# KumarRobotics/top_down_renderer

Hardware: AMD Instinct MI355X
Metric: particle-updates/sec (render+score+resample) (higher is better)
Workload: dtype f32

## Files before the change

### include/tdr.h

```cpp
#ifndef TDR_H_
#define TDR_H_

#include <stddef.h>
#include <stdint.h>

#ifdef __cplusplus
extern "C" {
#endif

#define TDR_OK 0
#define TDR_ERR_ARG (-1)
#define TDR_ERR_HIP (-2)
#define TDR_ERR_NOMEM (-3)

#define TDR_MAX_CLASSES 15
#define TDR_ST_FIELDS 7
enum { TDR_ST_INIT_X = 0, TDR_ST_INIT_Y = 1, TDR_ST_DX = 2, TDR_ST_DY = 3, TDR_ST_THETA = 4, TDR_ST_SCALE = 5,
       TDR_ST_HAVE_INIT = 6 };

typedef struct tdr_state {
  float init_x_px, init_y_px, dx_m, dy_m, theta, scale;
  uint8_t have_init;
  uint8_t pad_[3];
} tdr_state;
// ... 114 lines not shown
int tdr_k_score_cart_init(const tdr_map_desc* map, const float* scan_pk, int rows, int cols, float res,
                          const tdr_filter_params* fp, float* st, int64_t cap, int64_t n, int64_t n_total,
                          float* workspace, void* stream);

int tdr_k_propagate(float* st, int64_t cap, int64_t n, float* last_dist, float tx, float ty, float omega,
                    int scale_freeze, float pos_cov, float theta_cov, const float* z4, uint64_t seed, uint64_t step,
                    int64_t index_base, void* stream);
void* tdr_rng_create(uint32_t seed);
void tdr_rng_destroy(void* rng);
float tdr_rng_uniform_host(void* rng);
int tdr_propagate_normals_host(void* rng, int64_t n, int scale_freeze, float* z4_out);
#define TDR_RNG_STATE_WORDS 640
size_t tdr_rng_dev_workspace_bytes(int64_t n);
int tdr_k_rng_propagate_normals(uint32_t* state, int64_t n, int64_t lo, int64_t hi, int scale_freeze, float* z4_out,
                                void* workspace, void* stream);
int tdr_k_rng_uniform(uint32_t* state, float* out_dev, void* stream);
int tdr_rng_get_state_host(void* rng, uint32_t* words);
int tdr_rng_set_state_host(void* rng, const uint32_t* words);
typedef struct tdr_rng_pipe tdr_rng_pipe;
int tdr_rng_pipe_create(int64_t n_max, tdr_rng_pipe** out);
void tdr_rng_pipe_destroy(tdr_rng_pipe* p);
int tdr_rng_pipe_on_device(const tdr_rng_pipe* p);
int tdr_rng_pipe_from_host(tdr_rng_pipe* p, void* host_rng, void* stream);
int tdr_rng_pipe_to_host(tdr_rng_pipe* p, void* host_rng, void* stream);
int tdr_rng_pipe_normals(tdr_rng_pipe* p, int64_t n, int64_t lo, int64_t hi, int scale_freeze, const float** z4_out,
                         void* stream);
int tdr_rng_pipe_uniform(tdr_rng_pipe* p, const float** shift_out, void* stream);
int tdr_init_particle_host(void* rng, const float* class_maps, int ncls, int rows, int cols, float resolution,
                           const tdr_filter_params* fp, tdr_state* out);
int tdr_init_particles_host(void* rng, const float* class_maps, int ncls, int rows, int cols, float resolution,
                            const tdr_filter_params* fp, int max_num, tdr_state* out, int64_t* n_out);
int64_t tdr_init_particles_count(const tdr_filter_params* fp, int max_num);
size_t tdr_init_workspace_bytes(void);
int tdr_k_init_particles(uint32_t* rng_state_dev, const tdr_map_desc* map, const tdr_filter_params* fp, int max_num,
                         int64_t lo, int64_t hi, float* st, int64_t cap, int64_t* n_out, void* workspace, void* stream);
int tdr_rng_pipe_init_particles(tdr_rng_pipe* p, const tdr_map_desc* map, const tdr_filter_params* fp, int max_num,
                                int64_t lo, int64_t hi, float* st, int64_t cap, int64_t* n_out, void* workspace,
                                void* stream);

#define TDR_UW_INFO_FLOATS 65536
int tdr_k_update_weights(const float* raw_w, const float* last_dist, int64_t n, float* w_out, float* info_out,
                         void* stream);

int tdr_config_prefix_small(int on);
int64_t tdr_prefix_workspace_bytes(int64_t n);
int tdr_k_prefix(const float* w, int64_t n, float* runmax_out, void* workspace, void* stream);
int tdr_k_prefix_mode(const float* w, int64_t n, int mode, float* runmax_out, float* prefix_out, void* workspace,
// ... 270 lines not shown
```

### top_down_renderer_amd/_lib.py

```python
import ctypes as C
import os

_PKG = os.path.dirname(os.path.abspath(__file__))
SO_PATH = os.environ.get("TDR_LIB_PATH") or os.path.join(_PKG, "libtdr_hip.so")

TDR_ST_FIELDS = 7
TDR_MAX_CLASSES = 15
TDR_SVG_NO_KEY = 0xFFFFFFFF


class FilterParamsC(C.Structure):
    _fields_ = [
        ("pos_cov", C.c_float), ("theta_cov", C.c_float), ("regularization", C.c_float),
        ("init_pos_px_x", C.c_float), ("init_pos_px_y", C.c_float), ("init_pos_px_cov", C.c_float),
        ("init_pos_m_x", C.c_float), ("init_pos_m_y", C.c_float),
        ("init_pos_deg_theta", C.c_float), ("init_pos_deg_cov", C.c_float),
        ("force_on_map", C.c_int32),
        ("fixed_scale", C.c_float), ("scale_log_min", C.c_float), ("scale_log_max", C.c_float),
        ("num_classes", C.c_int32),
        ("class_weights", C.c_float * 16),
    ]


class MapDescC(C.Structure):
# ... 87 lines not shown
    "tdr_map_load_color_image": (_i, [_vp, _vp, _i, _i, _vp, _vp, _i, _i, _f, _i, _i]),
    "tdr_map_load_color_png": (_i, [_vp, C.c_char_p, _vp, _vp, _i, _i, _f, _i, _i]),
    "tdr_polygon_planes": (_i, [_vp, _vp, _vp, _i64, _i, _i, _i, _vp, _i, _f, _vp]),
    "tdr_k_unpack_map": (_i, [_vp, _i, _i, _i, _vp, _vp, _vp]),
    "tdr_polar_table_host": (_i, [_i, _i, _f, _f, _vp]),
    "tdr_raster_workspace_bytes": (_i64, [_i64]),
    "tdr_k_raster_polar": (_i, [_vp, _i, _i, _i64, _f, _f, _vp, _i, _i, _i, _vp, _vp, _vp, _vp]),
    "tdr_k_raster_cart": (_i, [_vp, _i, _i, _i64, _f, _vp, _i, _i, _i, _vp, _vp, _vp, _vp]),
    "tdr_raster_geo_workspace_bytes": (_i64, [_i64]),
    "tdr_k_raster_geo_polar": (_i, [_vp, _i, _i64, _i64, _f, _f, _i, _i, _vp, _vp, _vp]),
    "tdr_k_raster_geo_cart": (_i, [_vp, _i, _i64, _i64, _f, _i, _i, _vp, _vp]),
    "tdr_k_pack_scan": (_i, [_vp, _i, _i, _i, _vp, _vp]),
    "tdr_score_workspace_floats": (C.c_size_t, [_i, _i, _i, _i64, _i64]),
    "tdr_k_score_polar": (_i, [C.POINTER(MapDescC), _vp, _vp, _i, _i, _f, C.POINTER(FilterParamsC), _vp, _i64, _i64,
                               _i64, _vp, _f, _i, _vp, _vp, _vp]),
    "tdr_k_active_diffs": (_i, [C.POINTER(MapDescC), _vp, _i, _i, _f, _vp, _vp, _i, _i, _vp, _vp]),
    "tdr_active_candidates_host": (_i, [_vp, _i, _i, _vp, _vp, _vp, _vp, C.POINTER(_i), C.POINTER(_i)]),
    "tdr_logf_host": (_i, [_vp, _i64, _vp]),
    "tdr_k_selftest_logf": (_i, [_vp, _i64, _vp, _vp]),
    "tdr_rng_pipe_create": (_i, [_i64, C.POINTER(_vp)]),
    "tdr_rng_pipe_destroy": (None, [_vp]),
    "tdr_rng_pipe_on_device": (_i, [_vp]),
    "tdr_rng_pipe_from_host": (_i, [_vp, _vp, _vp]),
    "tdr_rng_pipe_to_host": (_i, [_vp, _vp, _vp]),
    "tdr_rng_pipe_normals": (_i, [_vp, _i64, _i64, _i64, _i, C.POINTER(_vp), _vp]),
    "tdr_rng_pipe_uniform": (_i, [_vp, C.POINTER(_vp), _vp]),
    "tdr_rng_dev_workspace_bytes": (C.c_size_t, [_i64]),
    "tdr_k_rng_propagate_normals": (_i, [_vp, _i64, _i64, _i64, _i, _vp, _vp, _vp]),
    "tdr_k_rng_uniform": (_i, [_vp, _vp, _vp]),
    "tdr_rng_get_state_host": (_i, [_vp, _vp]),
    "tdr_rng_set_state_host": (_i, [_vp, _vp]),
    "tdr_k_resample_dev": (_i, [_vp, _i64, _i64, _vp, _i64, _i64, _vp, _vp]),
    "tdr_score_ctx_create": (_i, [C.POINTER(_vp)]),
    "tdr_score_ctx_destroy": (None, [_vp]),
    "tdr_score_ctx_span": (C.c_float, [_vp]),
    "tdr_score_ctx_trial_calls": (_i64, [_vp]),
    "tdr_config_tuning": (_i64, [C.c_char_p, _i64]),
    "tdr_su_tail_plan": (_i, [_i, _i, _i, _i, C.POINTER(_i), C.POINTER(_i), C.POINTER(_i)]),
    "tdr_k_su_order_workspace_ints": (C.c_size_t, [_i64, _i]),
    "tdr_k_su_order_slots": (_i64, [_i64, _i]),
    "tdr_k_su_order": (_i, [_vp, _i64, _i64, _vp, _i, _f, _vp, _vp, _vp, _vp, C.POINTER(_i), _vp]),
    "tdr_k_score_prep": (_i, [_vp, _vp, _vp, _i, _i, _f, _vp, _i64, _i64, _i64, _vp, _f, _f, _vp, _vp, C.POINTER(_i64),
                              C.POINTER(_vp), _vp]),
    "tdr_selftest_score": (_i, []),
    "tdr_profile_variants": (_i, [C.POINTER(_i64)]),
    "tdr_score_ctx_set_polar_factors": (_i, [_vp, _vp, _i, _i]),
    "tdr_polar_factors_host": (_i, [_i, _i, _f, _f, _vp]),
# ... 173 lines not shown
```

### top_down_renderer_amd/csrc/tdr_rng.hip

```cpp
#include <rocprim/device/device_scan.hpp>

#include <random>
#include <sstream>

#include "tdr_common.h"
#include "tdr_mt_dev.h"
#include "tdr_mt_jump.h"

#define MT_N 624
#define MT_M 397

#define MT_X 1040
template <int S0, int NS>
__device__ __forceinline__ void mt_twist_batch(uint32_t* x, int lane, uint32_t* __restrict__ out) {
  uint32_t nv[NS];
#pragma unroll
  for (int s = 0; s < NS; s++) {
    const int k = 64 * (S0 + s) + lane;
    const int k1 = k == MT_N - 1 ? 0 : k + 1;
    const int si = k < MT_N - MT_M ? k + MT_M : k - (MT_N - MT_M);
    const uint32_t y = (x[k] & 0x80000000u) | (x[k1] & 0x7fffffffu);
    nv[s] = x[si] ^ (y >> 1) ^ ((0u - (y & 1u)) & 0x9908b0dfu);
  }
  __builtin_amdgcn_fence(__ATOMIC_RELEASE, "wavefront");
  __builtin_amdgcn_wave_barrier();
#pragma unroll
// ... 62 lines not shown
  }
  __syncthreads();
  if (wave != 0) return;
  for (int p = lane; p < MT_X; p += 64) xs[p] = p < MT_N ? R[MT_JUMP_CHUNKS - 1][p] : 0u;
  __builtin_amdgcn_fence(__ATOMIC_RELEASE, "wavefront");
  __builtin_amdgcn_wave_barrier();
  for (int j = MT_JUMP_CHUNKS - 2; j >= 0; j--) {
    mt_twist(xs, lane, nullptr);
    for (int p = lane; p < MT_N; p += 64) xs[p] ^= R[j][p];
    __builtin_amdgcn_fence(__ATOMIC_RELEASE, "wavefront");
    __builtin_amdgcn_wave_barrier();
  }
  if (lane == 0) {
    const uint32_t v = xs[MT_N - 1] ^ xs[MT_M - 1];
    const uint32_t lsb = v >> 31;
    const uint32_t y = ((v ^ (lsb ? 0x9908b0dfu : 0u)) << 1) | lsb;
    xs[0] = (xs[0] & 0x80000000u) | (y & 0x7fffffffu);
  }
  __builtin_amdgcn_fence(__ATOMIC_RELEASE, "wavefront");
  __builtin_amdgcn_wave_barrier();
  for (int p = lane; p < MT_N; p += 64) dst[p] = xs[p];
}

__global__ __launch_bounds__(256) void mt_attempt_kernel(const uint32_t* __restrict__ raw, const uint32_t* __restrict__ state,
                                                         int64_t nattempts, uint32_t* __restrict__ flags) {
  const int64_t t = (int64_t)blockIdx.x * blockDim.x + threadIdx.x;
  if (t >= nattempts) return;
  flags[t] = mt_attempt(raw, (int64_t)state[MT_N] + 2 * t).ok ? 1u : 0u;
}
__global__ __launch_bounds__(256) void mt_normal_kernel(const uint32_t* __restrict__ raw, const uint32_t* __restrict__ state,
                                                        const uint32_t* __restrict__ flags, const uint32_t* __restrict__ rank,
                                                        int64_t nattempts, int64_t n, int per, int64_t lo, int64_t hi,
                                                        float* __restrict__ z4, uint32_t* __restrict__ consumed) {
  const int64_t t = (int64_t)blockIdx.x * blockDim.x + threadIdx.x;
  if (t >= nattempts || !flags[t]) return;
  const int64_t a = rank[t];
  if (a >= n * per) return;
  if (a == n * per - 1) *consumed = (uint32_t)(2 * (t + 1));
  const int64_t p = a / per;
  const int slot = (int)(a - p * per);
  if (p < lo || p >= hi) return;
  const MtAttempt at = mt_attempt(raw, (int64_t)state[MT_N] + 2 * t);
  const float mult = mt_attempt_mult(at.r2);
  float* z = z4 + 4 * (p - lo);
  const float vy = at.y * mult * 1.f + 0.f, vx = at.x * mult * 1.f + 0.f;
  if (slot == 0) z[0] = vy;
  else if (slot == 1) { z[1] = vy; z[2] = vx; }
  else z[3] = vy;
  if (per == 2 && slot == 1) z[3] = 0.f;
}
__global__ __launch_bounds__(64) void mt_advance_kernel(const uint32_t* __restrict__ raw, int nblocks,
                                                        const uint32_t* __restrict__ consumed, uint32_t* __restrict__ state) {
  const uint32_t c = *consumed;
  if (c == 0xFFFFFFFFu) {
    if (threadIdx.x == 0) state[MT_N + 1] = 1u;
    return;
  }
  const int64_t q = (int64_t)state[MT_N] + c;
  int b = (int)(q / MT_N), p = (int)(q % MT_N);
  if (p == 0 && b > 0) { b--; p = MT_N; }
  if (b >= nblocks) {
    if (threadIdx.x == 0) state[MT_N + 1] = 1u;
    return;
  }
  uint32_t v[(MT_N + 63) / 64];
  for (int k = threadIdx.x, i = 0; k < MT_N; k += 64, i++) v[i] = raw[(int64_t)b * MT_N + k];
  for (int k = threadIdx.x, i = 0; k < MT_N; k += 64, i++) state[k] = v[i];
  if (threadIdx.x == 0) state[MT_N] = (uint32_t)p;
}
__global__ __launch_bounds__(64) void mt_uniform_kernel(uint32_t* __restrict__ state, float* __restrict__ out) {
  __shared__ uint32_t x[MT_X];
  const int lane = threadIdx.x;
  uint32_t p = state[MT_N];
  uint32_t word;
  if (p >= MT_N) {
    for (int k = lane; k < MT_N; k += 64) x[k] = state[k];
    __syncthreads();
    mt_twist(x, lane, state);
    p = 0;
    word = x[0];
  } else {
    word = state[p];
  }
  if (lane == 0) {
    *out = mt_canonical(mt_temper(word)) * (1.f - 0.f) + 0.f;
    state[MT_N] = p + 1;
  }
}

int tdr_mt_raw_stream(const uint32_t* state, int64_t nblocks, uint32_t* raw, hipStream_t s) {
  const int64_t nstretch = cdiv(nblocks, (int64_t)MT_JUMP_STRIDE);
  if (tdr_cfg().mt_stretches && nstretch > 1 && nstretch <= ((int64_t)1 << MT_JUMP_LEVELS)) {
    for (int m = 0; ((int64_t)1 << m) < nstretch; m++) {
      const int64_t have = (int64_t)1 << m, jumps = std::min(have, nstretch - have);
      hipLaunchKernelGGL(mt_jump_kernel, dim3((unsigned)jumps), dim3(1024), 0, s, state, raw, m);
      LAUNCH_CHECK("mt_jump");
    }
    hipLaunchKernelGGL(mt_fill_kernel, dim3((unsigned)nstretch), dim3(64), 0, s, state, (int)nblocks, MT_JUMP_STRIDE, raw);
  } else {
    hipLaunchKernelGGL(mt_fill_kernel, dim3(1), dim3(64), 0, s, state, (int)nblocks, (int)nblocks, raw);
  }
  LAUNCH_CHECK("mt_fill");
  return TDR_OK;
}
int tdr_mt_advance(const uint32_t* raw, int64_t nblocks, const uint32_t* consumed, uint32_t* state, hipStream_t s) {
  hipLaunchKernelGGL(mt_advance_kernel, dim3(1), dim3(64), 0, s, raw, (int)nblocks, consumed, state);
  LAUNCH_CHECK("mt_advance");
  return TDR_OK;
}
static int64_t mt_attempt_budget(int64_t need) {
  return (int64_t)std::ceil((double)need / 0.7853981633974483 * 1.05 + 12.0 * std::sqrt((double)need + 1.0) + 64.0);
}
static size_t mt_scan_bytes(int64_t nattempts) {
  size_t bytes = 0;
  uint32_t* p = nullptr;
  hipError_t e = rocprim::exclusive_scan(nullptr, bytes, p, p, 0u, (size_t)nattempts, rocprim::plus<uint32_t>(), (hipStream_t)0, false);
  if (e != hipSuccess || bytes == 0) bytes = (size_t)nattempts / 16 + 65536;
  return (bytes + 255) / 256 * 256;
}
struct MtWs {
  int64_t nattempts, nblocks;
  size_t off_flags, off_rank, off_scan, off_consumed, total;
};
static MtWs mt_ws(int64_t n, int per) {
  MtWs w;
  w.nattempts = mt_attempt_budget(n * per);
  w.nblocks = (2 * w.nattempts + MT_N) / MT_N + 2;
  size_t o = (size_t)w.nblocks * MT_N * 4;
  auto take = [&](size_t bytes) { const size_t at = o; o += (bytes + 255) / 256 * 256; return at; };
  o = (o + 255) / 256 * 256;
  w.off_flags = take((size_t)w.nattempts * 4);
  w.off_rank = take((size_t)w.nattempts * 4);
  w.off_scan = take(mt_scan_bytes(w.nattempts));
  w.off_consumed = take(256);
  w.total = o;
  return w;
}
extern "C" size_t tdr_rng_dev_workspace_bytes(int64_t n) {
  if (n < 1) n = 1;
  return mt_ws(n, 3).total;
}
extern "C" int tdr_k_rng_propagate_normals(uint32_t* state, int64_t n, int64_t lo, int64_t hi, int scale_freeze, float* z4_out,
                                           void* workspace, void* stream) {
  if (!state || !z4_out || !workspace) return fail(TDR_ERR_ARG, "rng_propagate_normals: null pointer");
  if (n < 1 || lo < 0 || hi > n || lo > hi) return fail(TDR_ERR_ARG, "rng_propagate_normals: bad range");
  hipStream_t s = (hipStream_t)stream;
  const int per = scale_freeze ? 2 : 3;
  const MtWs W = mt_ws(n, per);
  char* base = reinterpret_cast<char*>(workspace);
  uint32_t* raw = reinterpret_cast<uint32_t*>(base);
  uint32_t* flags = reinterpret_cast<uint32_t*>(base + W.off_flags);
  uint32_t* rank = reinterpret_cast<uint32_t*>(base + W.off_rank);
  uint32_t* consumed = reinterpret_cast<uint32_t*>(base + W.off_consumed);
  HIP_TRY(hipMemsetAsync(consumed, 0xFF, 4, s));
  if (int rc = tdr_mt_raw_stream(state, W.nblocks, raw, s)) return rc;
  const unsigned blocks = (unsigned)cdiv(W.nattempts, 256);
  hipLaunchKernelGGL(mt_attempt_kernel, dim3(blocks), dim3(256), 0, s, (const uint32_t*)raw, (const uint32_t*)state,
                     W.nattempts, flags);
  LAUNCH_CHECK("mt_attempt");
  size_t scan_bytes = mt_scan_bytes(W.nattempts);
  HIP_TRY(rocprim::exclusive_scan(base + W.off_scan, scan_bytes, flags, rank, 0u, (size_t)W.nattempts,
                                  rocprim::plus<uint32_t>(), s, false));
  hipLaunchKernelGGL(mt_normal_kernel, dim3(blocks), dim3(256), 0, s, (const uint32_t*)raw, (const uint32_t*)state,
                     (const uint32_t*)flags, (const uint32_t*)rank, W.nattempts, n, per, lo, hi, z4_out, consumed);
  LAUNCH_CHECK("mt_normal");
  return tdr_mt_advance(raw, W.nblocks, consumed, state, s);
}
extern "C" int tdr_k_rng_uniform(uint32_t* state, float* out, void* stream) {
  if (!state || !out) return fail(TDR_ERR_ARG, "rng_uniform: null pointer");
  hipLaunchKernelGGL(mt_uniform_kernel, dim3(1), dim3(64), 0, (hipStream_t)stream, state, out);
  LAUNCH_CHECK("mt_uniform");
  return TDR_OK;
}

extern "C" int tdr_rng_get_state_host(void* rng, uint32_t* words) {
  if (!rng || !words) return fail(TDR_ERR_ARG, "rng_get_state: null pointer");
  std::ostringstream os;
  os << *(std::mt19937*)rng;
  std::istringstream is(os.str());
  for (int k = 0; k <= MT_N; k++) {
    unsigned long long v = 0;
    if (!(is >> v)) return fail(TDR_ERR_ARG, "rng_get_state: unexpected engine format");
    words[k] = (uint32_t)v;
  }
  for (int k = MT_N + 1; k < TDR_RNG_STATE_WORDS; k++) words[k] = 0;
  return TDR_OK;
}
extern "C" int tdr_rng_set_state_host(void* rng, const uint32_t* words) {
  if (!rng || !words) return fail(TDR_ERR_ARG, "rng_set_state: null pointer");
// ... 4 lines not shown
  std::istringstream is(os.str());
  is >> *(std::mt19937*)rng;
  if (!is) return fail(TDR_ERR_ARG, "rng_set_state: the engine refused the state");
  return TDR_OK;
}

extern "C" int tdr_logf_host(const float* x, int64_t n, float* out) {
  if (!x || !out || n < 0) return fail(TDR_ERR_ARG, "logf_host: bad arguments");
  for (int64_t i = 0; i < n; i++) out[i] = tdr_libm::logf_t<true>(x[i]);
  return TDR_OK;
}
__global__ void selftest_logf_kernel(const float* __restrict__ x, int64_t n, float* __restrict__ out) {
  const int64_t i = (int64_t)blockIdx.x * blockDim.x + threadIdx.x;
  if (i < n) out[i] = tdr_libm::logf_t<true>(x[i]);
}
extern "C" int tdr_k_selftest_logf(const float* x, int64_t n, float* out, void* stream) {
  if (!x || !out || n < 0) return fail(TDR_ERR_ARG, "selftest_logf: bad arguments");
  if (n == 0) return TDR_OK;
  hipLaunchKernelGGL(selftest_logf_kernel, dim3((unsigned)cdiv(n, 256)), dim3(256), 0, (hipStream_t)stream, x, n, out);
  LAUNCH_CHECK("selftest_logf");
  return TDR_OK;
}

__global__ void mt_copy_kernel(const uint32_t* __restrict__ src, uint32_t* __restrict__ dst, int n, uint32_t* __restrict__ err) {
  const int k = blockIdx.x * blockDim.x + threadIdx.x;
  if (k < n) {
    const uint32_t v = src[k];
    if (dst) dst[k] = v;
    if (err && k == MT_N + 1 && v != 0) *err = v;
  }
}
static int mt_copy(const void* src, void* dst, int words, hipStream_t s, uint32_t* err = nullptr) {
  hipLaunchKernelGGL(mt_copy_kernel, dim3((unsigned)cdiv(words, 256)), dim3(256), 0, s, (const uint32_t*)src, (uint32_t*)dst, words, err);
  LAUNCH_CHECK("mt_copy");
  return TDR_OK;
}
struct tdr_rng_pipe {
  hipStream_t side = nullptr;
  hipEvent_t ev_fork = nullptr, ev_uniform = nullptr, ev_all = nullptr;
  uint32_t* state = nullptr;
  uint32_t* spec_state = nullptr;
  float* shift = nullptr;
  float* z[2] = {nullptr, nullptr};
  void* ws[2] = {nullptr, nullptr};
  int64_t n_max = 0;
  int cur = 0;
  bool on_device = false;
  int spec = 0;
  int64_t spec_n = 0, spec_lo = 0, spec_hi = 0;
  int spec_freeze = 0;
  int misses = 0;
  uint32_t* err_host = nullptr;
};
static int pipe_check(const tdr_rng_pipe* p, const char* who) {
  if (p->err_host && *(volatile const uint32_t*)p->err_host)
    return fail(TDR_ERR_HIP, "%s: an earlier call of the device generator ran out of its attempt budget — the stream is "
                             "stopped where it stood (probability ~1e-23 per call: more likely a damaged state)", who);
  return TDR_OK;
}
extern "C" int tdr_rng_pipe_create(int64_t n_max, tdr_rng_pipe** out) {
  if (!out || n_max < 1) return fail(TDR_ERR_ARG, "rng_pipe_create: bad arguments");
  *out = nullptr;
  tdr_rng_pipe* p = new (std::nothrow) tdr_rng_pipe;
  if (!p) return fail(TDR_ERR_NOMEM, "rng_pipe_create: out of memory");
  p->n_max = n_max;
  const size_t wsb = tdr_rng_dev_workspace_bytes(n_max);
  hipError_t e = hipStreamCreateWithFlags(&p->side, hipStreamNonBlocking);
  if (e == hipSuccess) e = hipEventCreateWithFlags(&p->ev_fork, hipEventDisableTiming);
  if (e == hipSuccess) e = hipEventCreateWithFlags(&p->ev_uniform, hipEventDisableTiming);
  if (e == hipSuccess) e = hipEventCreateWithFlags(&p->ev_all, hipEventDisableTiming);
  if (e == hipSuccess) e = hipMalloc((void**)&p->state, sizeof(uint32_t) * TDR_RNG_STATE_WORDS);
  if (e == hipSuccess) e = hipMalloc((void**)&p->spec_state, sizeof(uint32_t) * TDR_RNG_STATE_WORDS * 2);
  if (e == hipSuccess) e = hipMalloc((void**)&p->shift, sizeof(float) * 32);
  if (e == hipSuccess) e = hipHostMalloc((void**)&p->err_host, sizeof(uint32_t), hipHostMallocMapped);
  if (e == hipSuccess) *p->err_host = 0;
  for (int k = 0; k < 2 && e == hipSuccess; k++) {
    e = hipMalloc((void**)&p->z[k], sizeof(float) * 4 * (size_t)n_max);
    if (e == hipSuccess) e = hipMalloc(&p->ws[k], wsb);
  }
  if (e != hipSuccess) {
    tdr_rng_pipe_destroy(p);
    return fail(TDR_ERR_HIP, "rng_pipe_create: %s", hipGetErrorString(e));
  }
  *out = p;
  return TDR_OK;
}
extern "C" void tdr_rng_pipe_destroy(tdr_rng_pipe* p) {
  if (!p) return;
  if (p->side) { (void)hipStreamSynchronize(p->side); (void)hipStreamDestroy(p->side); }
  for (hipEvent_t ev : {p->ev_fork, p->ev_uniform, p->ev_all})
    if (ev) (void)hipEventDestroy(ev);
  (void)hipFree(p->state); (void)hipFree(p->spec_state); (void)hipFree(p->shift);
  if (p->err_host) (void)hipHostFree(p->err_host);
  for (int k = 0; k < 2; k++) { (void)hipFree(p->z[k]); (void)hipFree(p->ws[k]); }
  delete p;
}
extern "C" int tdr_rng_pipe_on_device(const tdr_rng_pipe* p) { return p && p->on_device ? 1 : 0; }
static int pipe_drop(tdr_rng_pipe* p, hipStream_t s) {
  if (!p->spec) return TDR_OK;
  HIP_TRY(hipStreamWaitEvent(s, p->ev_all, 0));
  if (p->spec == 2)
    if (int rc = mt_copy(p->spec_state + TDR_RNG_STATE_WORDS, p->state, TDR_RNG_STATE_WORDS, s)) return rc;
  p->spec = 0;
  return TDR_OK;
}
static int pipe_draw_ahead(tdr_rng_pipe* p, int64_t n, int64_t lo, int64_t hi, int freeze, hipStream_t s) {
  if (p->misses >= 2) return TDR_OK;
  HIP_TRY(hipEventRecord(p->ev_fork, s));
  HIP_TRY(hipStreamWaitEvent(p->side, p->ev_fork, 0));
  if (int rc = mt_copy(p->state, p->spec_state, TDR_RNG_STATE_WORDS, p->side)) return rc;
  if (int rc = tdr_k_rng_uniform(p->spec_state, p->shift + 16, p->side)) return rc;
  if (int rc = mt_copy(p->spec_state, p->spec_state + TDR_RNG_STATE_WORDS, TDR_RNG_STATE_WORDS, p->side)) return rc;
  HIP_TRY(hipEventRecord(p->ev_uniform, p->side));
  if (int rc = tdr_k_rng_propagate_normals(p->spec_state, n, lo, hi, freeze, p->z[1 - p->cur], p->ws[1 - p->cur], p->side)) return rc;
  HIP_TRY(hipEventRecord(p->ev_all, p->side));
  p->spec = 1;
  p->spec_n = n; p->spec_lo = lo; p->spec_hi = hi; p->spec_freeze = freeze;
  return TDR_OK;
}
extern "C" int tdr_rng_pipe_from_host(tdr_rng_pipe* p, void* host_rng, void* stream) {
  if (!p || !host_rng) return fail(TDR_ERR_ARG, "rng_pipe_from_host: null pointer");
  hipStream_t s = (hipStream_t)stream;
  if (int rc = pipe_drop(p, s)) return rc;
  uint32_t words[TDR_RNG_STATE_WORDS];
  if (int rc = tdr_rng_get_state_host(host_rng, words)) return rc;
  HIP_TRY(hipMemcpyAsync(p->state, words, sizeof(words), hipMemcpyHostToDevice, s));
  HIP_TRY(hipStreamSynchronize(s));
  p->on_device = true;
  p->misses = 0;
  if (p->err_host) *p->err_host = 0;
  return TDR_OK;
}
extern "C" int tdr_rng_pipe_to_host(tdr_rng_pipe* p, void* host_rng, void* stream) {
  if (!p || !host_rng) return fail(TDR_ERR_ARG, "rng_pipe_to_host: null pointer");
  if (!p->on_device) return TDR_OK;
  hipStream_t s = (hipStream_t)stream;
  if (int rc = pipe_drop(p, s)) return rc;
  uint32_t words[TDR_RNG_STATE_WORDS];
  HIP_TRY(hipMemcpyAsync(words, p->state, sizeof(words), hipMemcpyDeviceToHost, s));
  HIP_TRY(hipStreamSynchronize(s));
  if (int rc = tdr_rng_set_state_host(host_rng, words)) return rc;
  p->on_device = false;
  return TDR_OK;
}
extern "C" int tdr_rng_pipe_normals(tdr_rng_pipe* p, int64_t n, int64_t lo, int64_t hi, int scale_freeze, const float** z4_out,
                                    void* stream) {
  if (!p || !z4_out) return fail(TDR_ERR_ARG, "rng_pipe_normals: null pointer");
  if (!p->on_device) return fail(TDR_ERR_ARG, "rng_pipe_normals: the stream is on the host (tdr_rng_pipe_from_host)");
  if (n < 1 || n > p->n_max || lo < 0 || hi > n || lo > hi) return fail(TDR_ERR_ARG, "rng_pipe_normals: bad range");
  if (int rc = pipe_check(p, "rng_pipe_normals")) return rc;
  hipStream_t s = (hipStream_t)stream;
  const int fr = scale_freeze ? 1 : 0;
  if (p->spec == 2 && p->spec_n == n && p->spec_lo == lo && p->spec_hi == hi && p->spec_freeze == fr) {
    HIP_TRY(hipStreamWaitEvent(s, p->ev_all, 0));
    if (int rc = mt_copy(p->spec_state, p->state, TDR_RNG_STATE_WORDS, s, p->err_host)) return rc;
    p->cur = 1 - p->cur;
    p->spec = 0;
    p->misses = 0;
  } else {
    if (p->spec) p->misses++;
    else if (p->misses) p->misses--;
    if (int rc = pipe_drop(p, s)) return rc;
    if (int rc = tdr_k_rng_propagate_normals(p->state, n, lo, hi, fr, p->z[p->cur], p->ws[p->cur], s)) return rc;
    if (int rc = mt_copy(p->state, nullptr, TDR_RNG_STATE_WORDS, s, p->err_host)) return rc;
  }
  *z4_out = p->z[p->cur];
  return pipe_draw_ahead(p, n, lo, hi, fr, s);
}
extern "C" int tdr_rng_pipe_init_particles(tdr_rng_pipe* p, const tdr_map_desc* map, const tdr_filter_params* fp, int max_num,
                                           int64_t lo, int64_t hi, float* st, int64_t cap, int64_t* n_out, void* workspace,
                                           void* stream) {
  if (!p) return fail(TDR_ERR_ARG, "rng_pipe_init_particles: null pointer");
  if (!p->on_device) return fail(TDR_ERR_ARG, "rng_pipe_init_particles: the stream is on the host (tdr_rng_pipe_from_host)");
  if (int rc = pipe_check(p, "rng_pipe_init_particles")) return rc;
  hipStream_t s = (hipStream_t)stream;
  if (int rc = pipe_drop(p, s)) return rc;
  p->misses = 0;
  return tdr_k_init_particles(p->state, map, fp, max_num, lo, hi, st, cap, n_out, workspace, stream);
}
extern "C" int tdr_rng_pipe_uniform(tdr_rng_pipe* p, const float** shift_out, void* stream) {
  if (!p || !shift_out) return fail(TDR_ERR_ARG, "rng_pipe_uniform: null pointer");
  if (!p->on_device) return fail(TDR_ERR_ARG, "rng_pipe_uniform: the stream is on the host (tdr_rng_pipe_from_host)");
  if (int rc = pipe_check(p, "rng_pipe_uniform")) return rc;
  hipStream_t s = (hipStream_t)stream;
  if (p->spec == 1) {
    HIP_TRY(hipStreamWaitEvent(s, p->ev_uniform, 0));
    if (int rc = mt_copy(p->shift + 16, p->shift, 1, s)) return rc;
    p->spec = 2;
  } else {
    if (p->spec) p->misses++;
    if (int rc = pipe_drop(p, s)) return rc;
    if (int rc = tdr_k_rng_uniform(p->state, p->shift, s)) return rc;
  }
  *shift_out = p->shift;
  return TDR_OK;
}
```

### top_down_renderer_amd/kernels.py

```python
import ctypes as C

import numpy as np
import torch

from . import _lib
from ._lib import FilterParamsC, MapDescC, check


def _ptr(t):
    return C.c_void_p(t.data_ptr()) if t is not None else C.c_void_p(0)


class ScoreCtx:

    def __init__(self, lib, handle):
        self.lib, self.handle = lib, handle

    def span(self):
        return float(self.lib.tdr_score_ctx_span(self.handle))

    def trial_calls(self):
        return int(self.lib.tdr_score_ctx_trial_calls(self.handle))

    def __del__(self):
# ... 7 lines not shown

class DevPtr:

    def __init__(self, addr):
        self.addr = addr

    def data_ptr(self):
        return self.addr


class RngPipe:

    def __init__(self, kernels, handle):
        self.k, self.lib, self.handle = kernels, kernels.lib, handle

    def on_device(self):
        return bool(self.lib.tdr_rng_pipe_on_device(self.handle))

    def from_host(self, rng):
        check(self.lib.tdr_rng_pipe_from_host(self.handle, rng, self.k.stream()))

    def to_host(self, rng):
        check(self.lib.tdr_rng_pipe_to_host(self.handle, rng, self.k.stream()))

    def normals(self, n, lo, hi, scale_freeze):
        z = C.c_void_p(0)
        check(self.lib.tdr_rng_pipe_normals(self.handle, n, lo, hi, int(scale_freeze), C.byref(z), self.k.stream()))
        return DevPtr(z.value)

    def uniform(self):
        u = C.c_void_p(0)
        check(self.lib.tdr_rng_pipe_uniform(self.handle, C.byref(u), self.k.stream()))
        return DevPtr(u.value)

    def init_particles(self, dmap, fp, max_num, lo, hi, st):
        n = C.c_int64(0)
        ws = self.k.empty((int(self.lib.tdr_init_workspace_bytes()),), torch.uint8)
        check(self.lib.tdr_rng_pipe_init_particles(self.handle, C.byref(dmap.desc), C.byref(fp), max_num, lo, hi, _ptr(st),
                                                   st.shape[1], C.byref(n), _ptr(ws), self.k.stream()))
        return n.value

    def __del__(self):
        try:
            if self.handle:
                self.lib.tdr_rng_pipe_destroy(self.handle)
                self.handle = None
# ... 710 lines not shown
```

Baseline: 24.31 million.

## Fuse MT normal draw into count/rank kernels and swap RNG state buffers

Replaces the attempt-flag kernel, rocprim exclusive scan and separate advance step with workgroup-local ballot ranking. Each block finds its global offset either by recounting earlier attempts (small grids) or from per-block counts with group atomics. The normal kernel now also advances the state itself. The speculative pipe swaps indices into a triple state buffer instead of running copy kernels, and one fused kernel does the uniform step, snapshot and control-word arming. The aim is fewer kernel launches and less global scratch traffic on the RNG path. In exchange it adds redundant recounting work in the self-count path and more complex buffer-ownership logic.

```diff
diff --git a/include/tdr.h b/include/tdr.h
--- a/include/tdr.h
+++ b/include/tdr.h
@@ -160,7 +160,9 @@
 void tdr_rng_pipe_destroy(tdr_rng_pipe* p);
 int tdr_rng_pipe_on_device(const tdr_rng_pipe* p);
 int tdr_rng_pipe_from_host(tdr_rng_pipe* p, void* host_rng, void* stream);
+int tdr_rng_pipe_from_words(tdr_rng_pipe* p, const uint32_t* words, void* stream);
 int tdr_rng_pipe_to_host(tdr_rng_pipe* p, void* host_rng, void* stream);
+int tdr_rng_pipe_launches(const tdr_rng_pipe* p, int64_t* on_caller, int64_t* on_side);
 int tdr_rng_pipe_normals(tdr_rng_pipe* p, int64_t n, int64_t lo, int64_t hi, int scale_freeze, const float** z4_out,
                          void* stream);
 int tdr_rng_pipe_uniform(tdr_rng_pipe* p, const float** shift_out, void* stream);
diff --git a/top_down_renderer_amd/_lib.py b/top_down_renderer_amd/_lib.py
--- a/top_down_renderer_amd/_lib.py
+++ b/top_down_renderer_amd/_lib.py
@@ -133,7 +133,9 @@
     "tdr_rng_pipe_destroy": (None, [_vp]),
     "tdr_rng_pipe_on_device": (_i, [_vp]),
     "tdr_rng_pipe_from_host": (_i, [_vp, _vp, _vp]),
+    "tdr_rng_pipe_from_words": (_i, [_vp, _vp, _vp]),
     "tdr_rng_pipe_to_host": (_i, [_vp, _vp, _vp]),
+    "tdr_rng_pipe_launches": (_i, [_vp, C.POINTER(_i64), C.POINTER(_i64)]),
     "tdr_rng_pipe_normals": (_i, [_vp, _i64, _i64, _i64, _i, C.POINTER(_vp), _vp]),
     "tdr_rng_pipe_uniform": (_i, [_vp, C.POINTER(_vp), _vp]),
     "tdr_rng_dev_workspace_bytes": (C.c_size_t, [_i64]),
diff --git a/top_down_renderer_amd/csrc/tdr_rng.hip b/top_down_renderer_amd/csrc/tdr_rng.hip
--- a/top_down_renderer_amd/csrc/tdr_rng.hip
+++ b/top_down_renderer_amd/csrc/tdr_rng.hip
@@ -1,7 +1,6 @@
-#include <rocprim/device/device_scan.hpp>
-
 #include <random>
 #include <sstream>
+#include <utility>
 
 #include "tdr_common.h"
 #include "tdr_mt_dev.h"
@@ -110,32 +109,115 @@
   for (int p = lane; p < MT_N; p += 64) dst[p] = xs[p];
 }
 
-__global__ __launch_bounds__(256) void mt_attempt_kernel(const uint32_t* __restrict__ raw, const uint32_t* __restrict__ state,
-                                                         int64_t nattempts, uint32_t* __restrict__ flags) {
-  const int64_t t = (int64_t)blockIdx.x * blockDim.x + threadIdx.x;
-  if (t >= nattempts) return;
-  flags[t] = mt_attempt(raw, (int64_t)state[MT_N] + 2 * t).ok ? 1u : 0u;
-}
-__global__ __launch_bounds__(256) void mt_normal_kernel(const uint32_t* __restrict__ raw, const uint32_t* __restrict__ state,
-                                                        const uint32_t* __restrict__ flags, const uint32_t* __restrict__ rank,
-                                                        int64_t nattempts, int64_t n, int per, int64_t lo, int64_t hi,
-                                                        float* __restrict__ z4, uint32_t* __restrict__ consumed) {
-  const int64_t t = (int64_t)blockIdx.x * blockDim.x + threadIdx.x;
-  if (t >= nattempts || !flags[t]) return;
-  const int64_t a = rank[t];
-  if (a >= n * per) return;
-  if (a == n * per - 1) *consumed = (uint32_t)(2 * (t + 1));
-  const int64_t p = a / per;
-  const int slot = (int)(a - p * per);
-  if (p < lo || p >= hi) return;
-  const MtAttempt at = mt_attempt(raw, (int64_t)state[MT_N] + 2 * t);
-  const float mult = mt_attempt_mult(at.r2);
-  float* z = z4 + 4 * (p - lo);
-  const float vy = at.y * mult * 1.f + 0.f, vx = at.x * mult * 1.f + 0.f;
-  if (slot == 0) z[0] = vy;
-  else if (slot == 1) { z[1] = vy; z[2] = vx; }
-  else z[3] = vy;
-  if (per == 2 && slot == 1) z[3] = 0.f;
+#define MT_ITEMS 4
+#define MT_WG_ATTEMPTS (256 * MT_ITEMS)
+#define MT_GROUP 64
+#define MT_SELF_COUNT_WGS 128
+#define MT_CTL_GROUPS 2
+__device__ __forceinline__ uint32_t mt_wg_ranks(const uint32_t* __restrict__ raw, int64_t p0, int64_t t0, int64_t nattempts,
+                                                MtAttempt (&at)[MT_ITEMS], uint32_t& ok, uint32_t (&base)[MT_ITEMS]) {
+  __shared__ uint32_t part[MT_ITEMS][4];
+  const int tid = threadIdx.x, lane = tid & 63, wave = tid >> 6;
+  ok = 0;
+  uint64_t bal[MT_ITEMS];
+#pragma unroll
+  for (int j = 0; j < MT_ITEMS; j++) {
+    const int64_t t = t0 + 256 * j + tid;
+    bool acc = false;
+    if (t < nattempts) {
+      at[j] = mt_attempt(raw, p0 + 2 * t);
+      acc = at[j].ok;
+    }
+    bal[j] = __ballot(acc);
+    if (acc) ok |= 1u << j;
+    if (lane == 0) part[j][wave] = (uint32_t)__popcll(bal[j]);
+  }
+  __syncthreads();
+  uint32_t run = 0;
+#pragma unroll
+  for (int j = 0; j < MT_ITEMS; j++) {
+#pragma unroll
+    for (int w = 0; w < 4; w++) {
+      if (w == wave) base[j] = run + (uint32_t)__popcll(bal[j] & (((uint64_t)1 << lane) - 1));
+      run += part[j][w];
+    }
+  }
+  return run;
+}
+__global__ __launch_bounds__(256) void mt_count_kernel(const uint32_t* __restrict__ raw, int64_t nattempts,
+                                                       uint32_t* __restrict__ counts, uint32_t* __restrict__ ctl) {
+  MtAttempt at[MT_ITEMS];
+  uint32_t ok, base[MT_ITEMS];
+  const uint32_t total = mt_wg_ranks(raw, (int64_t)ctl[1], (int64_t)blockIdx.x * MT_WG_ATTEMPTS, nattempts, at, ok, base);
+  if (threadIdx.x == 0) {
+    counts[blockIdx.x] = total;
+    atomicAdd(&ctl[MT_CTL_GROUPS + blockIdx.x / MT_GROUP], total);
+  }
+}
+template <bool SELF_COUNT>
+__global__ __launch_bounds__(256) void mt_normal_kernel(const uint32_t* __restrict__ raw, int nblocks, uint32_t* __restrict__ state,
+                                                        const uint32_t* __restrict__ counts, int64_t nattempts, int64_t n, int per,
+                                                        int64_t lo, int64_t hi, float* __restrict__ z4, uint32_t* __restrict__ ctl,
+                                                        uint32_t* __restrict__ err) {
+  __shared__ uint32_t front[4];
+  __shared__ uint32_t fin;
+  const int tid = threadIdx.x, lane = tid & 63, wave = tid >> 6;
+  const int64_t p0 = ctl[1];
+  uint32_t acc = 0;
+  if (SELF_COUNT) {
+    for (int64_t t = tid; t < (int64_t)blockIdx.x * MT_WG_ATTEMPTS; t += 256) acc += mt_attempt(raw, p0 + 2 * t).ok ? 1u : 0u;
+  } else {
+    const int g = blockIdx.x / MT_GROUP;
+    for (int i = tid; i < g; i += 256) acc += ctl[MT_CTL_GROUPS + i];
+    if (tid < (int)blockIdx.x - g * MT_GROUP) acc += counts[g * MT_GROUP + tid];
+  }
+#pragma unroll
+  for (int o = 32; o > 0; o >>= 1) acc += __shfl_xor(acc, o);
+  if (lane == 0) front[wave] = acc;
+  if (tid == 0) fin = 0xFFFFFFFFu;
+  __syncthreads();
+  const int64_t first = (int64_t)front[0] + front[1] + front[2] + front[3];
+  if (first >= n * per) return;
+  MtAttempt at[MT_ITEMS];
+  uint32_t ok, base[MT_ITEMS];
+  const uint32_t total = mt_wg_ranks(raw, p0, (int64_t)blockIdx.x * MT_WG_ATTEMPTS, nattempts, at, ok, base);
+#pragma unroll
+  for (int j = 0; j < MT_ITEMS; j++) {
+    if (!(ok >> j & 1u)) continue;
+    const int64_t t = (int64_t)blockIdx.x * MT_WG_ATTEMPTS + 256 * j + tid;
+    const int64_t a = first + base[j];
+    if (a >= n * per) continue;
+    if (a == n * per - 1) fin = (uint32_t)(2 * (t + 1));
+    const int64_t p = a / per;
+    const int slot = (int)(a - p * per);
+    if (p < lo || p >= hi) continue;
+    const float mult = mt_attempt_mult(at[j].r2);
+    float* z = z4 + 4 * (p - lo);
+    const float vy = at[j].y * mult * 1.f + 0.f, vx = at[j].x * mult * 1.f + 0.f;
+    if (slot == 0) z[0] = vy;
+    else if (slot == 1) { z[1] = vy; z[2] = vx; }
+    else z[3] = vy;
+    if (per == 2 && slot == 1) z[3] = 0.f;
+  }
+  __syncthreads();
+  const uint32_t c = fin;
+  bool raise = false;
+  if (c != 0xFFFFFFFFu) {
+    const int64_t q = p0 + c;
+    int b = (int)(q / MT_N), p = (int)(q % MT_N);
+    if (p == 0 && b > 0) { b--; p = MT_N; }
+    if (b >= nblocks) raise = true;
+    else {
+      for (int k = tid; k < MT_N; k += 256) state[k] = raw[(int64_t)b * MT_N + k];
+      if (tid == 0) { state[MT_N] = (uint32_t)p; ctl[0] = c; }
+    }
+  } else if (blockIdx.x == gridDim.x - 1 && first + total < n * per) {
+    raise = true;
+  }
+  if (raise && tid == 0) { state[MT_N + 1] = 1u; if (err) *err = 1u; }
+}
+__global__ __launch_bounds__(64) void mt_arm_kernel(const uint32_t* __restrict__ state, uint32_t* __restrict__ ctl, int nctl) {
+  for (int i = threadIdx.x; i < nctl; i += 64) ctl[i] = i == 0 ? 0xFFFFFFFFu : i == 1 ? state[MT_N] : 0u;
 }
 __global__ __launch_bounds__(64) void mt_advance_kernel(const uint32_t* __restrict__ raw, int nblocks,
                                                         const uint32_t* __restrict__ consumed, uint32_t* __restrict__ state) {
@@ -175,6 +257,33 @@
     state[MT_N] = p + 1;
   }
 }
+__global__ __launch_bounds__(64) void mt_uniform_step_kernel(const uint32_t* __restrict__ real, uint32_t* __restrict__ snap,
+                                                             uint32_t* __restrict__ work, float* __restrict__ out,
+                                                             uint32_t* __restrict__ ctl, int nctl, uint32_t* __restrict__ err_snap,
+                                                             uint32_t* __restrict__ err_work) {
+  __shared__ uint32_t x[MT_X];
+  const int lane = threadIdx.x;
+  uint32_t p = real[MT_N];
+  for (int k = lane; k < MT_N; k += 64) x[k] = real[k];
+  __syncthreads();
+  if (p >= MT_N) {
+    mt_twist(x, lane, nullptr);
+    p = 0;
+  }
+  for (int k = lane; k < MT_N; k += 64) {
+    const uint32_t v = x[k];
+    snap[k] = v;
+    work[k] = v;
+  }
+  for (int i = lane; i < nctl; i += 64) ctl[i] = i == 0 ? 0xFFFFFFFFu : i == 1 ? p + 1 : 0u;
+  if (lane == 0) {
+    *out = mt_canonical(mt_temper(x[p])) * (1.f - 0.f) + 0.f;
+    const uint32_t e = real[MT_N + 1];
+    snap[MT_N] = p + 1; work[MT_N] = p + 1;
+    snap[MT_N + 1] = e; work[MT_N + 1] = e;
+    if (e != 0) { *err_snap = e; *err_work = e; }
+  }
+}
 
 int tdr_mt_raw_stream(const uint32_t* state, int64_t nblocks, uint32_t* raw, hipStream_t s) {
   const int64_t nstretch = cdiv(nblocks, (int64_t)MT_JUMP_STRIDE);
@@ -199,60 +308,72 @@
 static int64_t mt_attempt_budget(int64_t need) {
   return (int64_t)std::ceil((double)need / 0.7853981633974483 * 1.05 + 12.0 * std::sqrt((double)need + 1.0) + 64.0);
 }
-static size_t mt_scan_bytes(int64_t nattempts) {
-  size_t bytes = 0;
-  uint32_t* p = nullptr;
-  hipError_t e = rocprim::exclusive_scan(nullptr, bytes, p, p, 0u, (size_t)nattempts, rocprim::plus<uint32_t>(), (hipStream_t)0, false);
-  if (e != hipSuccess || bytes == 0) bytes = (size_t)nattempts / 16 + 65536;
-  return (bytes + 255) / 256 * 256;
-}
 struct MtWs {
-  int64_t nattempts, nblocks;
-  size_t off_flags, off_rank, off_scan, off_consumed, total;
+  int64_t nattempts, nblocks, nwg;
+  int nctl;
+  size_t off_counts, off_ctl, total;
 };
 static MtWs mt_ws(int64_t n, int per) {
   MtWs w;
   w.nattempts = mt_attempt_budget(n * per);
   w.nblocks = (2 * w.nattempts + MT_N) / MT_N + 2;
+  w.nwg = cdiv(w.nattempts, (int64_t)MT_WG_ATTEMPTS);
+  w.nctl = MT_CTL_GROUPS + (int)cdiv(w.nwg, (int64_t)MT_GROUP);
   size_t o = (size_t)w.nblocks * MT_N * 4;
   auto take = [&](size_t bytes) { const size_t at = o; o += (bytes + 255) / 256 * 256; return at; };
   o = (o + 255) / 256 * 256;
-  w.off_flags = take((size_t)w.nattempts * 4);
-  w.off_rank = take((size_t)w.nattempts * 4);
-  w.off_scan = take(mt_scan_bytes(w.nattempts));
-  w.off_consumed = take(256);
+  w.off_counts = take((size_t)w.nwg * 4);
+  w.off_ctl = take((size_t)w.nctl * 4);
   w.total = o;
   return w;
+}
+static int mt_raw_stream_launches(int64_t nblocks) {
+  const int64_t nstretch = cdiv(nblocks, (int64_t)MT_JUMP_STRIDE);
+  int k = 1;
+  if (tdr_cfg().mt_stretches && nstretch > 1 && nstretch <= ((int64_t)1 << MT_JUMP_LEVELS))
+    for (int m = 0; ((int64_t)1 << m) < nstretch; m++) k++;
+  return k;
 }
 extern "C" size_t tdr_rng_dev_workspace_bytes(int64_t n) {
   if (n < 1) n = 1;
   return mt_ws(n, 3).total;
+}
+static uint32_t* mt_ws_ctl(void* workspace, int64_t n, int per, int* nctl) {
+  const MtWs W = mt_ws(n, per);
+  *nctl = W.nctl;
+  return reinterpret_cast<uint32_t*>(reinterpret_cast<char*>(workspace) + W.off_ctl);
+}
+static int mt_propagate_normals(uint32_t* state, int64_t n, int64_t lo, int64_t hi, int per, float* z4_out, void* workspace,
+                                bool armed, uint32_t* err, int64_t* launches, hipStream_t s) {
+  const MtWs W = mt_ws(n, per);
+  char* base = reinterpret_cast<char*>(workspace);
+  uint32_t* raw = reinterpret_cast<uint32_t*>(base);
+  uint32_t* counts = reinterpret_cast<uint32_t*>(base + W.off_counts);
+  uint32_t* ctl = reinterpret_cast<uint32_t*>(base + W.off_ctl);
+  if (!armed) {
+    hipLaunchKernelGGL(mt_arm_kernel, dim3(1), dim3(64), 0, s, (const uint32_t*)state, ctl, W.nctl);
+    LAUNCH_CHECK("mt_arm");
+  }
+  if (int rc = tdr_mt_raw_stream(state, W.nblocks, raw, s)) return rc;
+  const bool self_count = W.nwg <= MT_SELF_COUNT_WGS;
+  if (self_count) {
+    hipLaunchKernelGGL(mt_normal_kernel<true>, dim3((unsigned)W.nwg), dim3(256), 0, s, (const uint32_t*)raw, (int)W.nblocks, state,
+                       (const uint32_t*)counts, W.nattempts, n, per, lo, hi, z4_out, ctl, err);
+  } else {
+    hipLaunchKernelGGL(mt_count_kernel, dim3((unsigned)W.nwg), dim3(256), 0, s, (const uint32_t*)raw, W.nattempts, counts, ctl);
+    LAUNCH_CHECK("mt_count");
+    hipLaunchKernelGGL(mt_normal_kernel<false>, dim3((unsigned)W.nwg), dim3(256), 0, s, (const uint32_t*)raw, (int)W.nblocks, state,
+                       (const uint32_t*)counts, W.nattempts, n, per, lo, hi, z4_out, ctl, err);
+  }
+  LAUNCH_CHECK("mt_normal");
+  if (launches) *launches += (armed ? 0 : 1) + mt_raw_stream_launches(W.nblocks) + (self_count ? 1 : 2);
+  return TDR_OK;
 }
 extern "C" int tdr_k_rng_propagate_normals(uint32_t* state, int64_t n, int64_t lo, int64_t hi, int scale_freeze, float* z4_out,
                                            void* workspace, void* stream) {
   if (!state || !z4_out || !workspace) return fail(TDR_ERR_ARG, "rng_propagate_normals: null pointer");
   if (n < 1 || lo < 0 || hi > n || lo > hi) return fail(TDR_ERR_ARG, "rng_propagate_normals: bad range");
-  hipStream_t s = (hipStream_t)stream;
-  const int per = scale_freeze ? 2 : 3;
-  const MtWs W = mt_ws(n, per);
-  char* base = reinterpret_cast<char*>(workspace);
-  uint32_t* raw = reinterpret_cast<uint32_t*>(base);
-  uint32_t* flags = reinterpret_cast<uint32_t*>(base + W.off_flags);
-  uint32_t* rank = reinterpret_cast<uint32_t*>(base + W.off_rank);
-  uint32_t* consumed = reinterpret_cast<uint32_t*>(base + W.off_consumed);
-  HIP_TRY(hipMemsetAsync(consumed, 0xFF, 4, s));
-  if (int rc = tdr_mt_raw_stream(state, W.nblocks, raw, s)) return rc;
-  const unsigned blocks = (unsigned)cdiv(W.nattempts, 256);
-  hipLaunchKernelGGL(mt_attempt_kernel, dim3(blocks), dim3(256), 0, s, (const uint32_t*)raw, (const uint32_t*)state,
-                     W.nattempts, flags);
-  LAUNCH_CHECK("mt_attempt");
-  size_t scan_bytes = mt_scan_bytes(W.nattempts);
-  HIP_TRY(rocprim::exclusive_scan(base + W.off_scan, scan_bytes, flags, rank, 0u, (size_t)W.nattempts,
-                                  rocprim::plus<uint32_t>(), s, false));
-  hipLaunchKernelGGL(mt_normal_kernel, dim3(blocks), dim3(256), 0, s, (const uint32_t*)raw, (const uint32_t*)state,
-                     (const uint32_t*)flags, (const uint32_t*)rank, W.nattempts, n, per, lo, hi, z4_out, consumed);
-  LAUNCH_CHECK("mt_normal");
-  return tdr_mt_advance(raw, W.nblocks, consumed, state, s);
+  return mt_propagate_normals(state, n, lo, hi, scale_freeze ? 2 : 3, z4_out, workspace, false, nullptr, nullptr, (hipStream_t)stream);
 }
 extern "C" int tdr_k_rng_uniform(uint32_t* state, float* out, void* stream) {
   if (!state || !out) return fail(TDR_ERR_ARG, "rng_uniform: null pointer");
@@ -303,25 +424,13 @@
   return TDR_OK;
 }
 
-__global__ void mt_copy_kernel(const uint32_t* __restrict__ src, uint32_t* __restrict__ dst, int n, uint32_t* __restrict__ err) {
-  const int k = blockIdx.x * blockDim.x + threadIdx.x;
-  if (k < n) {
-    const uint32_t v = src[k];
-    if (dst) dst[k] = v;
-    if (err && k == MT_N + 1 && v != 0) *err = v;
-  }
-}
-static int mt_copy(const void* src, void* dst, int words, hipStream_t s, uint32_t* err = nullptr) {
-  hipLaunchKernelGGL(mt_copy_kernel, dim3((unsigned)cdiv(words, 256)), dim3(256), 0, s, (const uint32_t*)src, (uint32_t*)dst, words, err);
-  LAUNCH_CHECK("mt_copy");
-  return TDR_OK;
-}
 struct tdr_rng_pipe {
   hipStream_t side = nullptr;
-  hipEvent_t ev_fork = nullptr, ev_uniform = nullptr, ev_all = nullptr;
-  uint32_t* state = nullptr;
-  uint32_t* spec_state = nullptr;
+  hipEvent_t ev_fork = nullptr, ev_all = nullptr;
+  uint32_t* sbuf = nullptr;
+  int real = 0, work = 1, snap = 2;
   float* shift = nullptr;
+  int ucur = 0;
   float* z[2] = {nullptr, nullptr};
   void* ws[2] = {nullptr, nullptr};
   int64_t n_max = 0;
@@ -331,10 +440,14 @@
   int64_t spec_n = 0, spec_lo = 0, spec_hi = 0;
   int spec_freeze = 0;
   int misses = 0;
+  hipStream_t waited = nullptr;
   uint32_t* err_host = nullptr;
+  int64_t on_caller = 0, on_side = 0;
+  uint32_t* st(int k) const { return sbuf + (size_t)k * TDR_RNG_STATE_WORDS; }
+  float* slot(int k) const { return shift + 16 * k; }
 };
 static int pipe_check(const tdr_rng_pipe* p, const char* who) {
-  if (p->err_host && *(volatile const uint32_t*)p->err_host)
+  if (p->err_host && *(volatile const uint32_t*)(p->err_host + p->real))
     return fail(TDR_ERR_HIP, "%s: an earlier call of the device generator ran out of its attempt budget — the stream is "
                              "stopped where it stood (probability ~1e-23 per call: more likely a damaged state)", who);
   return TDR_OK;
@@ -348,13 +461,11 @@
   const size_t wsb = tdr_rng_dev_workspace_bytes(n_max);
   hipError_t e = hipStreamCreateWithFlags(&p->side, hipStreamNonBlocking);
   if (e == hipSuccess) e = hipEventCreateWithFlags(&p->ev_fork, hipEventDisableTiming);
-  if (e == hipSuccess) e = hipEventCreateWithFlags(&p->ev_uniform, hipEventDisableTiming);
   if (e == hipSuccess) e = hipEventCreateWithFlags(&p->ev_all, hipEventDisableTiming);
-  if (e == hipSuccess) e = hipMalloc((void**)&p->state, sizeof(uint32_t) * TDR_RNG_STATE_WORDS);
-  if (e == hipSuccess) e = hipMalloc((void**)&p->spec_state, sizeof(uint32_t) * TDR_RNG_STATE_WORDS * 2);
+  if (e == hipSuccess) e = hipMalloc((void**)&p->sbuf, sizeof(uint32_t) * TDR_RNG_STATE_WORDS * 3);
   if (e == hipSuccess) e = hipMalloc((void**)&p->shift, sizeof(float) * 32);
-  if (e == hipSuccess) e = hipHostMalloc((void**)&p->err_host, sizeof(uint32_t), hipHostMallocMapped);
-  if (e == hipSuccess) *p->err_host = 0;
+  if (e == hipSuccess) e = hipHostMalloc((void**)&p->err_host, sizeof(uint32_t) * 3, hipHostMallocMapped);
+  if (e == hipSuccess) p->err_host[0] = p->err_host[1] = p->err_host[2] = 0;
   for (int k = 0; k < 2 && e == hipSuccess; k++) {
     e = hipMalloc((void**)&p->z[k], sizeof(float) * 4 * (size_t)n_max);
     if (e == hipSuccess) e = hipMalloc(&p->ws[k], wsb);
@@ -369,31 +480,42 @@
 extern "C" void tdr_rng_pipe_destroy(tdr_rng_pipe* p) {
   if (!p) return;
   if (p->side) { (void)hipStreamSynchronize(p->side); (void)hipStreamDestroy(p->side); }
-  for (hipEvent_t ev : {p->ev_fork, p->ev_uniform, p->ev_all})
+  for (hipEvent_t ev : {p->ev_fork, p->ev_all})
     if (ev) (void)hipEventDestroy(ev);
-  (void)hipFree(p->state); (void)hipFree(p->spec_state); (void)hipFree(p->shift);
+  (void)hipFree(p->sbuf); (void)hipFree(p->shift);
   if (p->err_host) (void)hipHostFree(p->err_host);
   for (int k = 0; k < 2; k++) { (void)hipFree(p->z[k]); (void)hipFree(p->ws[k]); }
   delete p;
 }
 extern "C" int tdr_rng_pipe_on_device(const tdr_rng_pipe* p) { return p && p->on_device ? 1 : 0; }
+extern "C" int tdr_rng_pipe_launches(const tdr_rng_pipe* p, int64_t* on_caller, int64_t* on_side) {
+  if (!p) return fail(TDR_ERR_ARG, "rng_pipe_launches: null pointer");
+  if (on_caller) *on_caller = p->on_caller;
+  if (on_side) *on_side = p->on_side;
+  return TDR_OK;
+}
 static int pipe_drop(tdr_rng_pipe* p, hipStream_t s) {
   if (!p->spec) return TDR_OK;
   HIP_TRY(hipStreamWaitEvent(s, p->ev_all, 0));
-  if (p->spec == 2)
-    if (int rc = mt_copy(p->spec_state + TDR_RNG_STATE_WORDS, p->state, TDR_RNG_STATE_WORDS, s)) return rc;
+  if (p->spec == 2) std::swap(p->real, p->snap);
   p->spec = 0;
   return TDR_OK;
 }
 static int pipe_draw_ahead(tdr_rng_pipe* p, int64_t n, int64_t lo, int64_t hi, int freeze, hipStream_t s) {
   if (p->misses >= 2) return TDR_OK;
+  const int per = freeze ? 2 : 3;
+  void* ws = p->ws[1 - p->cur];
+  int nctl = 0;
+  uint32_t* ctl = mt_ws_ctl(ws, n, per, &nctl);
   HIP_TRY(hipEventRecord(p->ev_fork, s));
   HIP_TRY(hipStreamWaitEvent(p->side, p->ev_fork, 0));
-  if (int rc = mt_copy(p->state, p->spec_state, TDR_RNG_STATE_WORDS, p->side)) return rc;
-  if (int rc = tdr_k_rng_uniform(p->spec_state, p->shift + 16, p->side)) return rc;
-  if (int rc = mt_copy(p->spec_state, p->spec_state + TDR_RNG_STATE_WORDS, TDR_RNG_STATE_WORDS, p->side)) return rc;
-  HIP_TRY(hipEventRecord(p->ev_uniform, p->side));
-  if (int rc = tdr_k_rng_propagate_normals(p->spec_state, n, lo, hi, freeze, p->z[1 - p->cur], p->ws[1 - p->cur], p->side)) return rc;
+  p->err_host[p->work] = p->err_host[p->snap] = 0;
+  hipLaunchKernelGGL(mt_uniform_step_kernel, dim3(1), dim3(64), 0, p->side, (const uint32_t*)p->st(p->real), p->st(p->snap),
+                     p->st(p->work), p->slot(1 - p->ucur), ctl, nctl, p->err_host + p->snap, p->err_host + p->work);
+  LAUNCH_CHECK("mt_uniform_step");
+  p->on_side++;
+  if (int rc = mt_propagate_normals(p->st(p->work), n, lo, hi, per, p->z[1 - p->cur], ws, true, p->err_host + p->work,
+                                    &p->on_side, p->side)) return rc;
   HIP_TRY(hipEventRecord(p->ev_all, p->side));
   p->spec = 1;
   p->spec_n = n; p->spec_lo = lo; p->spec_hi = hi; p->spec_freeze = freeze;
@@ -401,15 +523,20 @@
 }
 extern "C" int tdr_rng_pipe_from_host(tdr_rng_pipe* p, void* host_rng, void* stream) {
   if (!p || !host_rng) return fail(TDR_ERR_ARG, "rng_pipe_from_host: null pointer");
+  uint32_t words[TDR_RNG_STATE_WORDS];
+  if (int rc = tdr_rng_get_state_host(host_rng, words)) return rc;
+  return tdr_rng_pipe_from_words(p, words, stream);
+}
+extern "C" int tdr_rng_pipe_from_words(tdr_rng_pipe* p, const uint32_t* words, void* stream) {
+  if (!p || !words) return fail(TDR_ERR_ARG, "rng_pipe_from_words: null pointer");
+  if (words[MT_N] > MT_N) return fail(TDR_ERR_ARG, "rng_pipe_from_words: index %u", words[MT_N]);
   hipStream_t s = (hipStream_t)stream;
   if (int rc = pipe_drop(p, s)) return rc;
-  uint32_t words[TDR_RNG_STATE_WORDS];
-  if (int rc = tdr_rng_get_state_host(host_rng, words)) return rc;
-  HIP_TRY(hipMemcpyAsync(p->state, words, sizeof(words), hipMemcpyHostToDevice, s));
+  HIP_TRY(hipMemcpyAsync(p->st(p->real), words, sizeof(uint32_t) * TDR_RNG_STATE_WORDS, hipMemcpyHostToDevice, s));
   HIP_TRY(hipStreamSynchronize(s));
   p->on_device = true;
   p->misses = 0;
-  if (p->err_host) *p->err_host = 0;
+  p->err_host[p->real] = words[MT_N + 1];
   return TDR_OK;
 }
 extern "C" int tdr_rng_pipe_to_host(tdr_rng_pipe* p, void* host_rng, void* stream) {
@@ -418,7 +545,7 @@
   hipStream_t s = (hipStream_t)stream;
   if (int rc = pipe_drop(p, s)) return rc;
   uint32_t words[TDR_RNG_STATE_WORDS];
-  HIP_TRY(hipMemcpyAsync(words, p->state, sizeof(words), hipMemcpyDeviceToHost, s));
+  HIP_TRY(hipMemcpyAsync(words, p->st(p->real), sizeof(words), hipMemcpyDeviceToHost, s));
   HIP_TRY(hipStreamSynchronize(s));
   if (int rc = tdr_rng_set_state_host(host_rng, words)) return rc;
   p->on_device = false;
@@ -433,8 +560,8 @@
   hipStream_t s = (hipStream_t)stream;
   const int fr = scale_freeze ? 1 : 0;
   if (p->spec == 2 && p->spec_n == n && p->spec_lo == lo && p->spec_hi == hi && p->spec_freeze == fr) {
-    HIP_TRY(hipStreamWaitEvent(s, p->ev_all, 0));
-    if (int rc = mt_copy(p->spec_state, p->state, TDR_RNG_STATE_WORDS, s, p->err_host)) return rc;
+    if (s != p->waited) HIP_TRY(hipStreamWaitEvent(s, p->ev_all, 0));
+    std::swap(p->real, p->work);
     p->cur = 1 - p->cur;
     p->spec = 0;
     p->misses = 0;
@@ -442,8 +569,8 @@
     if (p->spec) p->misses++;
     else if (p->misses) p->misses--;
     if (int rc = pipe_drop(p, s)) return rc;
-    if (int rc = tdr_k_rng_propagate_normals(p->state, n, lo, hi, fr, p->z[p->cur], p->ws[p->cur], s)) return rc;
-    if (int rc = mt_copy(p->state, nullptr, TDR_RNG_STATE_WORDS, s, p->err_host)) return rc;
+    if (int rc = mt_propagate_normals(p->st(p->real), n, lo, hi, fr ? 2 : 3, p->z[p->cur], p->ws[p->cur], false,
+                                      p->err_host + p->real, &p->on_caller, s)) return rc;
   }
   *z4_out = p->z[p->cur];
   return pipe_draw_ahead(p, n, lo, hi, fr, s);
@@ -457,7 +584,7 @@
   hipStream_t s = (hipStream_t)stream;
   if (int rc = pipe_drop(p, s)) return rc;
   p->misses = 0;
-  return tdr_k_init_particles(p->state, map, fp, max_num, lo, hi, st, cap, n_out, workspace, stream);
+  return tdr_k_init_particles(p->st(p->real), map, fp, max_num, lo, hi, st, cap, n_out, workspace, stream);
 }
 extern "C" int tdr_rng_pipe_uniform(tdr_rng_pipe* p, const float** shift_out, void* stream) {
   if (!p || !shift_out) return fail(TDR_ERR_ARG, "rng_pipe_uniform: null pointer");
@@ -465,14 +592,16 @@
   if (int rc = pipe_check(p, "rng_pipe_uniform")) return rc;
   hipStream_t s = (hipStream_t)stream;
   if (p->spec == 1) {
-    HIP_TRY(hipStreamWaitEvent(s, p->ev_uniform, 0));
-    if (int rc = mt_copy(p->shift + 16, p->shift, 1, s)) return rc;
+    HIP_TRY(hipStreamWaitEvent(s, p->ev_all, 0));
+    p->waited = s;
     p->spec = 2;
   } else {
     if (p->spec) p->misses++;
     if (int rc = pipe_drop(p, s)) return rc;
-    if (int rc = tdr_k_rng_uniform(p->state, p->shift, s)) return rc;
-  }
-  *shift_out = p->shift;
-  return TDR_OK;
-}
+    if (int rc = tdr_k_rng_uniform(p->st(p->real), p->slot(1 - p->ucur), s)) return rc;
+    p->on_caller++;
+  }
+  p->ucur = 1 - p->ucur;
+  *shift_out = p->slot(p->ucur);
+  return TDR_OK;
+}
diff --git a/top_down_renderer_amd/kernels.py b/top_down_renderer_amd/kernels.py
--- a/top_down_renderer_amd/kernels.py
+++ b/top_down_renderer_amd/kernels.py
@@ -53,6 +53,14 @@
 
     def to_host(self, rng):
         check(self.lib.tdr_rng_pipe_to_host(self.handle, rng, self.k.stream()))
+
+    def from_words(self, words):
+        check(self.lib.tdr_rng_pipe_from_words(self.handle, words.ctypes.data_as(C.c_void_p), self.k.stream()))
+
+    def launches(self):
+        a, b = C.c_int64(0), C.c_int64(0)
+        check(self.lib.tdr_rng_pipe_launches(self.handle, C.byref(a), C.byref(b)))
+        return a.value, b.value
 
     def normals(self, n, lo, hi, scale_freeze):
         z = C.c_void_p(0)
```

After: 24.43 million (median of 6 runs). Within noise of the previous version (+0.5%).
